# too-z/MultiModalPFN

Hardware: NVIDIA B200
Metric: test rows/sec predict_proba (higher is better)
Workload: dtype bf16

## Files before the change

### multimodalpfn_b200/csrc/common.cuh

```cuda
#pragma once
#include <cuda_bf16.h>
#include <cuda_runtime.h>
#include <stdint.h>

#include <atomic>

#include "../../include/mmpfn_b200.h"

namespace mmpfn {

constexpr int kE = 192;
constexpr int kH = 6;
constexpr int kD = 32;
constexpr int kHid = 768;
constexpr float kLnEps = 1e-5f;

extern std::atomic<int64_t> g_launches;
void set_error(const char* fmt, ...);
int check_geometry(const mmpfn_geometry* g);

inline int count_launch() {
  g_launches.fetch_add(1, std::memory_order_relaxed);
  cudaError_t e = cudaGetLastError();
  if (e != cudaSuccess) {
// ... 4 lines not shown
}

inline int current_device() {
  int d = 0;
  if (cudaGetDevice(&d) != cudaSuccess) { cudaGetLastError(); return -1; }
  return d;
}
inline int device_sm_count() {
  static int n[64] = {0};
  const int d = current_device();
  if (d < 0 || d >= 64) return 148;
  if (!n[d]) {
    int v = 0;
    if (cudaDeviceGetAttribute(&v, cudaDevAttrMultiProcessorCount, d) != cudaSuccess || v < 1) { cudaGetLastError(); v = 148; }
    n[d] = v;
  }
  return n[d];
}
#define MMPFN_OPT_IN_SMEM(kern, bytes)                                                                     \
  do {                                                                                                     \
    static unsigned long long _done = 0;                                                                   \
    const int _d = ::mmpfn::current_device();                                                              \
    if (_d < 0 || _d >= 64 || !((_done >> _d) & 1ull)) {                                                   \
      if (cudaFuncSetAttribute(kern, cudaFuncAttributeMaxDynamicSharedMemorySize, (int)(bytes)) != cudaSuccess) { \
        ::mmpfn::set_error("cannot opt in to %d bytes of dynamic shared memory: %s", (int)(bytes),           \
                           cudaGetErrorString(cudaGetLastError()));                                        \
        return MMPFN_ECUDA;                                                                                \
      }                                                                                                    \
      if (_d >= 0 && _d < 64) _done |= 1ull << _d;                                                         \
    }                                                                                                      \
  } while (0)

#define MMPFN_TRY(expr)            \
  do {                             \
    int _rc = (expr);              \
    if (_rc != MMPFN_OK) return _rc; \
  } while (0)

__device__ __forceinline__ float gelu_exact(float x) {
  return 0.5f * x * (1.0f + erff(x * 0.70710678118654752440f));
}
__device__ __forceinline__ float warp_sum(float v) {
#pragma unroll
  for (int o = 16; o > 0; o >>= 1) v += __shfl_xor_sync(0xffffffffu, v, o);
  return v;
}
__device__ __forceinline__ float warp_max(float v) {
#pragma unroll
  for (int o = 16; o > 0; o >>= 1) v = fmaxf(v, __shfl_xor_sync(0xffffffffu, v, o));
  return v;
}
__device__ __forceinline__ uint32_t pack_bf16x2(float lo, float hi) {
  __nv_bfloat162 v = __floats2bfloat162_rn(lo, hi);
  return *reinterpret_cast<uint32_t*>(&v);
}
__device__ __forceinline__ float fast_exp2f(float x) {
  float y;
  asm("ex2.approx.ftz.f32 %0, %1;" : "=f"(y) : "f"(x));
  return y;
}
__device__ __forceinline__ float bf16_bits_to_float(uint16_t b) { return __uint_as_float(uint32_t(b) << 16); }

enum { EPI_NONE = 0, EPI_GELU = 1, EPI_GLU_PAIR = 2, EPI_ADD_C = 3 };

struct SgemmParams {
  const float* A;
  const float* W;
  const float* bias;
  float* C;
  int M, N, K, lda, ldw, ldc;
  long long a_batch, w_batch, bias_batch, c_batch;
  int batches;
  int row_inner, row_outer;
};
int launch_sgemm(const SgemmParams& p, int epi, cudaStream_t st);

int launch_layernorm(const float* x, const float* res, const float* gamma, const float* beta, long long rows,
                     int width, float* y_f32, uint16_t* y_bf16, cudaStream_t st, long long x_stride = 0);
int launch_kv_extract_f32(const float* qkv, float* kv, int B, int S, int T, cudaStream_t st, const int* n_rows = nullptr);

int launch_feat_attn_f32(const float* qkv, float* att, long long n_seq, int T, cudaStream_t st);
int launch_feat_attn_bf16(const uint16_t* qkv, uint16_t* att, long long n_seq, int T, cudaStream_t st);
bool feat_qkv_attn_supported(int T);
int launch_feat_qkv_attn(const uint16_t* x, const uint16_t* w_qkv, long long M, int T, uint16_t* att, cudaStream_t st);

struct ItemAttnF32 {
  const float *q, *k, *v;
  float* out;
  long long q_outer, q_inner, q_row, kv_outer, kv_inner, kv_row, o_outer, o_inner, o_row;
  int planes, inner, n_q, n_kv, shared_kv;
  const int *q_len, *kv_len;
};
int launch_item_attn_f32(const ItemAttnF32& p, cudaStream_t st);

enum { TC_EPI_BF16 = 0, TC_EPI_GELU_BF16 = 1, TC_EPI_RESID_LN = 2, TC_EPI_QKV_ITEMS = 3, TC_EPI_GLU_PAIR_F32 = 4 };
struct TcGemm {
  const uint16_t* A;
  const uint16_t* W;
  int M, N, K;
  int items;
  int B, S, T;
  int epi;
  uint16_t* out_bf16;
  float* resid_f32;
  uint16_t* ln_bf16;
  uint16_t *q_out, *k_out, *vt_out;
  int S_pad;
  uint16_t *k0_out, *vt0_out;
  const float* bias;
  float* out_f32;
};
int launch_tc_gemm(const TcGemm& p, cudaStream_t st);
int launch_tc_rowgemm(const TcGemm& p, cudaStream_t st);

struct TcMlp {
  const uint16_t* state_b;
  uint16_t* state_b_out;
  float* resid_f32;
  const uint16_t* w1;
  const uint16_t* w2;
  int M;
};
int launch_tc_mlp(const TcMlp& p, cudaStream_t st);

struct TcItemAttn {
  const uint16_t* q;
  const uint16_t* k;
  const uint16_t* vt;
  uint16_t* out;
  int B, T, n_q, Sq_pad, n_kv, Skv_pad;
  int shared_kv;
  int kv_slots;
  long long kv_rank_stride;
  int kv_seg_rows;
  long long kv_seg_stride;
  const int* q_len;
  const int* kv_len;
};
int launch_tc_item_attn(const TcItemAttn& p, cudaStream_t st);

struct TabStatsLayout {
  int Fp, G;
  __host__ __device__ int src() const { return 0; }
  __host__ __device__ int fill() const { return Fp; }
  __host__ __device__ int lo() const { return 2 * Fp; }
  __host__ __device__ int hi() const { return 3 * Fp; }
  __host__ __device__ int mean() const { return 4 * Fp; }
  __host__ __device__ int stdv() const { return 5 * Fp; }
  __host__ __device__ int scale() const { return 6 * Fp; }
  __host__ __device__ int total() const { return 6 * Fp + G; }
};
int launch_tab_fit(const float* x, int B, int S, int F, int fpg, int n_train, float n_sigma, float* stats,
                   cudaStream_t st, const int* n_rows = nullptr, const int* n_train_b = nullptr);
int launch_stem_tokens(const mmpfn_geometry* g, const mmpfn_weights* w, const float* x, const float* stats,
                       const float* img_tok, const float* y, const float* y_mean, const uint64_t* y_mask,
                       const float* pos_emb, int B, int S, int F, int H_img, long long x_bstride, long long y_bstride,
                       long long img_bstride, float* state_f32, uint16_t* state_bf16, int32_t* nan_flag, cudaStream_t st,
                       const long long* img_off = nullptr, const int* n_rows = nullptr);
int launch_cap_attn(const float* kv, const float* q, int S, int n_kv, int Hc, float* out, cudaStream_t st);
int launch_cap_combine(const float* o, const float* ffn, const float* gamma, const float* beta, long long rows,
                       float* out, cudaStream_t st);
int launch_moe_gate_scale(const float* gate_logits, float* tok, int S, int Hm, cudaStream_t st);
int launch_proba_tail(const float* logits, const int32_t* perm, const float* prior, int n_est, int S, int n_out,
                      int n_classes, float temperature, int avg_before, float* proba, cudaStream_t st);

int launch_bar_tail(const float* logits, const float* const* task_logits, const int32_t* row_offset, int n_tasks,
// ... 6 lines not shown
```

### multimodalpfn_b200/csrc/kernels_f32.cu

```cuda
#include "common.cuh"
#include "feat_attn_core.cuh"

namespace mmpfn {

namespace {
constexpr int BM = 128, BN = 64, BK = 16;

template <int EPI>
__global__ void __launch_bounds__(256) sgemm_kernel(SgemmParams p) {
  __shared__ __align__(16) float As[BK][BM + 4];
  __shared__ __align__(16) float Bs[BK][BN + 4];
  const int z = blockIdx.z;
  const float* __restrict__ A = p.A + z * p.a_batch;
  const float* __restrict__ W = p.W + z * p.w_batch;
  const float* __restrict__ bias = p.bias ? p.bias + z * p.bias_batch : nullptr;
  float* __restrict__ C = p.C + z * p.c_batch;
  const int m0 = blockIdx.x * BM, n0 = blockIdx.y * BN;
  const int tid = threadIdx.x;
  const int ty = tid >> 4, tx = tid & 15;

  float acc[8][4];
#pragma unroll
  for (int i = 0; i < 8; ++i)
#pragma unroll
// ... 236 lines not shown
  const int warp = threadIdx.x >> 5, lane = threadIdx.x & 31;
  const int n_kt = (T + 15) >> 4;
  const int Tp = n_kt * 16;
  const uint32_t buf_bytes = (uint32_t)Tp * FA_ROW_BYTES;
  const uint32_t sbase0 = (uint32_t)__cvta_generic_to_shared(fsm);
  constexpr int CH = 3 * kE * 2 / 16;

  auto stage = [&](long long row, int b) {
    const uint8_t* src = reinterpret_cast<const uint8_t*>(qkv + row * T * (3 * kE));
    const uint32_t dst = sbase0 + b * buf_bytes;
    for (int i = threadIdx.x; i < T * CH; i += blockDim.x) {
      const int t = i / CH, c = i % CH;
      asm volatile("cp.async.cg.shared.global [%0], [%1], 16;" ::"r"(dst + t * FA_ROW_BYTES + c * 16),
                   "l"(src + (long long)t * (3 * kE * 2) + c * 16));
    }
    asm volatile("cp.async.commit_group;");
  };
  for (int b = 0; b < n_buf; ++b)
    for (int i = threadIdx.x; i < (Tp - T) * CH; i += blockDim.x) {
      const int t = T + i / CH, c = i % CH;
      *reinterpret_cast<uint4*>(fsm + b * buf_bytes + t * FA_ROW_BYTES + c * 16) = make_uint4(0, 0, 0, 0);
    }
  long long row = blockIdx.x;
  if (row < n_rows) stage(row, 0);
  for (int it = 0; row < n_rows; row += gridDim.x, ++it) {
  const int cur = n_buf == 2 ? (it & 1) : 0;
  const long long nxt = row + gridDim.x;
  if (n_buf == 2 && nxt < n_rows) {
    stage(nxt, cur ^ 1);
    asm volatile("cp.async.wait_group 1;");
  } else {
    asm volatile("cp.async.wait_group 0;");
  }
  __syncthreads();
  const uint32_t sbase = sbase0 + cur * buf_bytes;

  const int n_items = kH * n_kt;
  for (int item = warp; item < n_items; item += (blockDim.x >> 5)) {
    const int h = item / n_kt, mt = item % n_kt;
    feat_attn_item<KT>(sbase, FA_ROW_BYTES, h * kD * 2, (kE + h * kD) * 2, (2 * kE + h * kD) * 2, T, n_kt, mt, lane);
  }
  __syncthreads();
  {
    constexpr int OC = kE * 2 / 16;
    uint8_t* dst = reinterpret_cast<uint8_t*>(att + row * T * kE);
    for (int i = threadIdx.x; i < T * OC; i += blockDim.x) {
      const int t = i / OC, c = i % OC;
      uint4 v;
      asm volatile("ld.shared.v4.b32 {%0, %1, %2, %3}, [%4];" : "=r"(v.x), "=r"(v.y), "=r"(v.z), "=r"(v.w)
                   : "r"(sbase + t * FA_ROW_BYTES + c * 16));
      *reinterpret_cast<uint4*>(dst + (long long)t * (kE * 2) + c * 16) = v;
    }
  }
  __syncthreads();
  if (n_buf == 1 && nxt < n_rows) stage(nxt, 0);
  }
}

template <int KT>
int launch_feat_attn_mma_t(const uint16_t* qkv, uint16_t* att, long long n_seq, int T, cudaStream_t st) {
  const int Tp = (T + 15) / 16 * 16;
  const int n_buf = (size_t)2 * Tp * FA_ROW_BYTES <= 200 * 1024 ? 2 : 1;
  const size_t smem = (size_t)n_buf * Tp * FA_ROW_BYTES;
  auto kern = feat_attn_mma_kernel<KT>;
  MMPFN_OPT_IN_SMEM(kern, 227 * 1024);
  const int n_sm = device_sm_count();
  const int n_items = kH * (Tp / 16);
  const int warps = n_items < 12 ? n_items : 12;
  int per_sm = (int)((227 * 1024) / (smem + 1024));
  if (per_sm > 2048 / (warps * 32)) per_sm = 2048 / (warps * 32);
  if (per_sm < 1) per_sm = 1;
  long long grid = (long long)n_sm * per_sm;
  if (grid > n_seq) grid = n_seq;
  kern<<<(unsigned)grid, warps * 32, smem, st>>>(qkv, att, T, n_seq, n_buf);
  return count_launch();
}
}

int launch_feat_attn_f32(const float* qkv, float* att, long long n_seq, int T, cudaStream_t st) {
  return launch_feat_attn<float, float>(qkv, att, n_seq, T, st);
}
int launch_feat_attn_bf16(const uint16_t* qkv, uint16_t* att, long long n_seq, int T, cudaStream_t st) {
  if (n_seq <= 0) return MMPFN_OK;
  if (T <= 32) return launch_feat_attn_mma_t<2>(qkv, att, n_seq, T, st);
  if (T <= 64) return launch_feat_attn_mma_t<4>(qkv, att, n_seq, T, st);
  if (T <= 96) return launch_feat_attn_mma_t<6>(qkv, att, n_seq, T, st);
  if (T <= 144) return launch_feat_attn_mma_t<9>(qkv, att, n_seq, T, st);
  if (T <= 192) return launch_feat_attn_mma_t<12>(qkv, att, n_seq, T, st);
  return launch_feat_attn<uint16_t, uint16_t>(qkv, att, n_seq, T, st);
}

namespace {
constexpr int IQ = 64, IK = 64;

__global__ void __launch_bounds__(128) item_attn_f32_kernel(ItemAttnF32 p) {
  __shared__ __align__(16) float Qt[kD][IQ];
  __shared__ __align__(16) float Kt[kD][IK];
  __shared__ __align__(16) float Vs[IK][kD];
  __shared__ __align__(16) float Pt[IK][IQ + 4];
  const int plane = blockIdx.z, h = blockIdx.y, q0 = blockIdx.x * IQ;
  const int tid = threadIdx.x;
  const int ty = tid >> 3, tx = tid & 7;
  const int pb = plane / p.inner, pt = plane % p.inner;
  const float* qb = p.q + pb * p.q_outer + pt * p.q_inner + h * kD;
  const int hk = p.shared_kv ? 0 : h;
  const float* kb = p.k + pb * p.kv_outer + pt * p.kv_inner + hk * kD;
  const float* vb = p.v + pb * p.kv_outer + pt * p.kv_inner + hk * kD;
  const int n_q = p.q_len ? min(max(p.q_len[pb], 0), p.n_q) : p.n_q;
  const int n_kv = p.kv_len ? min(max(p.kv_len[pb], 1), p.n_kv) : p.n_kv;
  if (q0 >= n_q) {
    for (int i = tid; i < IQ * (kD / 4); i += 128) {
      const int r = q0 + (i >> 3), c4 = (i & 7) * 4;
      if (r < p.n_q)
        *reinterpret_cast<float4*>(p.out + pb * p.o_outer + pt * p.o_inner + (long long)r * p.o_row + h * kD + c4) =
            make_float4(0.f, 0.f, 0.f, 0.f);
    }
    return;
  }

  const float scale = 0.17677669529663687f;
  for (int i = tid; i < IQ * (kD / 4); i += 128) {
    const int r = i >> 3, c4 = (i & 7) * 4;
    float4 v = make_float4(0, 0, 0, 0);
    if (q0 + r < n_q) v = *reinterpret_cast<const float4*>(qb + (long long)(q0 + r) * p.q_row + c4);
    Qt[c4 + 0][r] = v.x * scale; Qt[c4 + 1][r] = v.y * scale; Qt[c4 + 2][r] = v.z * scale; Qt[c4 + 3][r] = v.w * scale;
  }
  float m[4], l[4], o[4][4];
#pragma unroll
  for (int i = 0; i < 4; ++i) {
    m[i] = -INFINITY;
    l[i] = 0.f;
#pragma unroll
    for (int j = 0; j < 4; ++j) o[i][j] = 0.f;
  }

  for (int k0 = 0; k0 < n_kv; k0 += IK) {
    __syncthreads();
    for (int i = tid; i < IK * (kD / 4); i += 128) {
      const int r = i >> 3, c4 = (i & 7) * 4;
      float4 kv = make_float4(0, 0, 0, 0), vv = kv;
      if (k0 + r < n_kv) {
        kv = *reinterpret_cast<const float4*>(kb + (long long)(k0 + r) * p.kv_row + c4);
        vv = *reinterpret_cast<const float4*>(vb + (long long)(k0 + r) * p.kv_row + c4);
      }
      Kt[c4 + 0][r] = kv.x; Kt[c4 + 1][r] = kv.y; Kt[c4 + 2][r] = kv.z; Kt[c4 + 3][r] = kv.w;
      *reinterpret_cast<float4*>(&Vs[r][c4]) = vv;
    }
    __syncthreads();
    float s[4][8];
#pragma unroll
    for (int i = 0; i < 4; ++i)
#pragma unroll
      for (int j = 0; j < 8; ++j) s[i][j] = 0.f;
#pragma unroll 8
    for (int d = 0; d < kD; ++d) {
      const float4 a = *reinterpret_cast<const float4*>(&Qt[d][ty * 4]);
      const float4 b0 = *reinterpret_cast<const float4*>(&Kt[d][tx * 8]);
      const float4 b1 = *reinterpret_cast<const float4*>(&Kt[d][tx * 8 + 4]);
      const float av[4] = {a.x, a.y, a.z, a.w};
      const float bv[8] = {b0.x, b0.y, b0.z, b0.w, b1.x, b1.y, b1.z, b1.w};
#pragma unroll
      for (int i = 0; i < 4; ++i)
#pragma unroll
        for (int j = 0; j < 8; ++j) s[i][j] = fmaf(av[i], bv[j], s[i][j]);
    }
    float alpha[4];
#pragma unroll
// ... 98 lines not shown
```

### multimodalpfn_b200/csrc/kernels_featfused.cu

```cuda
#include "feat_attn_core.cuh"
#include "tc_common.cuh"

namespace mmpfn {
namespace {

constexpr int U_BM = 128, U_BN = 192, U_K = 192;
constexpr int U_W_BYTES = U_BN * U_K * 2;
constexpr int U_A_BYTES = U_BM * U_K * 2;
constexpr int U_ROW = 2 * 3 * kD * 2 + 16;
constexpr int U_QKV_BYTES = U_BM * U_ROW;
constexpr int U_PAD_ROWS = 12;
constexpr int U_OFF_W = 0;
constexpr int U_OFF_A = U_W_BYTES;
constexpr int U_OFF_QKV = U_OFF_A + U_A_BYTES;
constexpr int U_OFF_BAR = U_OFF_QKV + 2 * U_QKV_BYTES + U_PAD_ROWS * U_ROW;
constexpr int U_SMEM = U_OFF_BAR + 128 + 1024;
constexpr int U_THREADS = 768;
static_assert(U_SMEM <= 227 * 1024, "shared memory budget");
static_assert(U_ROW % 16 == 0 && U_ROW % 128 == 16, "ldmatrix rows: 16-byte aligned, 16 bytes apart modulo 128");

struct FusedArgs {
  uint16_t* att;
  long long M;
  long long n_rows;
// ... 84 lines not shown
#pragma unroll
          for (int k = 0; k < 4; ++k)
            umma_bf16(tmem + ab * U_BN, adesc + (uint64_t)(k * 2), bdesc + (uint64_t)(k * 2), idesc, (kb | k) != 0);
        }
        umma_commit(a_empty);
        umma_commit(&acc_full[ab]);
      }
    }
  } else if (warp >= 4 && warp < 8) {
    const int quarter = warp & 3;
    const int r = quarter * 32 + lane;
    uint32_t v[32];
    for (int i = 0; i < my_tiles; ++i) {
      const int ab = i & 1;
      const uint32_t row = smem_u32(smem) + U_OFF_QKV + ab * U_QKV_BYTES + r * U_ROW;
      const uint32_t trow = tmem + ab * U_BN + ((uint32_t)(quarter * 32) << 16);
      mbar_wait(&acc_full[ab], (i >> 1) & 1);
      tc_fence_after();
#pragma unroll 1
      for (int h2 = 0; h2 < 2; ++h2) {
        mbar_wait(&qkv_empty[ab * 2 + h2], ((i >> 1) & 1) ^ 1);
#pragma unroll 1
        for (int part = 0; part < 3; ++part) {
          const int c = part * 2 + h2;
          tmem_ld32(trow + c * 32, v);
          tmem_ld_wait();
#pragma unroll
          for (int k = 0; k < 4; ++k)
            st_shared_v4(row + c * 64 + k * 16, pack_bf16x2(__uint_as_float(v[8 * k]), __uint_as_float(v[8 * k + 1])),
                         pack_bf16x2(__uint_as_float(v[8 * k + 2]), __uint_as_float(v[8 * k + 3])),
                         pack_bf16x2(__uint_as_float(v[8 * k + 4]), __uint_as_float(v[8 * k + 5])),
                         pack_bf16x2(__uint_as_float(v[8 * k + 6]), __uint_as_float(v[8 * k + 7])));
        }
        mbar_arrive_warp(&qkv_full[ab * 2 + h2]);
      }
      tc_fence_before();
      mbar_arrive_warp(&acc_empty[ab]);
    }
  } else if (warp >= 8) {
    const int h2 = (warp - 8) >> 3, aw = (warp - 8) & 7;
    const int n_kt = (p.T + 15) >> 4;
    for (int i = 0; i < my_tiles; ++i) {
      const int qb = i & 1;
      const uint32_t qbase = smem_u32(smem) + U_OFF_QKV + qb * U_QKV_BYTES;
      const long long row0 = (long long)tile_of(i) * p.G;
      const int g_valid = (int)(p.n_rows - row0 < p.G ? p.n_rows - row0 : p.G);
      mbar_wait(&qkv_full[qb * 2 + h2], (i >> 1) & 1);
      const int n_items = g_valid * n_kt;
      uint8_t* dst = reinterpret_cast<uint8_t*>(p.att + (row0 * p.T) * kE + pair * 64 + h2 * 32);
      for (int item = aw; item < n_items; item += 8) {
        const int g = item / n_kt, mt = item % n_kt;
        const uint32_t rbase = qbase + g * p.T * U_ROW;
        feat_attn_item<KT>(rbase, U_ROW, h2 * 64, 128 + h2 * 64, 256 + h2 * 64, p.T, n_kt, mt, lane);
        __syncwarp();
#pragma unroll
        for (int k = 0; k < 2; ++k) {
          const int idx = lane + 32 * k, t = mt * 16 + (idx >> 2), c = idx & 3;
          if (t < p.T) {
            uint4 o;
            asm volatile("ld.shared.v4.b32 {%0, %1, %2, %3}, [%4];" : "=r"(o.x), "=r"(o.y), "=r"(o.z), "=r"(o.w)
                         : "r"(rbase + t * U_ROW + h2 * 64 + c * 16));
            *reinterpret_cast<uint4*>(dst + (long long)(g * p.T + t) * (kE * 2) + c * 16) = o;
          }
        }
      }
      mbar_arrive_warp(&qkv_empty[qb * 2 + h2]);
    }
  }
  tc_fence_before();
  __syncthreads();
  if (warp == 2) {
    tc_fence_after();
    tmem_dealloc(tmem, 512);
  }
}

template <int KT>
int launch_fused_t(const CUtensorMap& ma, const CUtensorMap& mw, const FusedArgs& a, int grid, cudaStream_t st) {
  MMPFN_OPT_IN_SMEM(feat_qkv_attn_kernel<KT>, U_SMEM);
  feat_qkv_attn_kernel<KT><<<grid, U_THREADS, U_SMEM, st>>>(ma, mw, a);
  return count_launch();
}

}

bool feat_qkv_attn_supported(int T) { return T >= 2 && T <= 64; }

int launch_feat_qkv_attn(const uint16_t* x, const uint16_t* w_qkv, long long M, int T, uint16_t* att, cudaStream_t st) {
  if (M <= 0) return MMPFN_OK;
  if (!feat_qkv_attn_supported(T) || M % T != 0 || M > 2147483647LL) {
    set_error("feat_qkv_attn: unsupported shape (M %lld, T %d)", M, T);
    return MMPFN_EUNSUPPORTED;
  }
  FusedArgs a{};
  a.att = att; a.M = M; a.T = T; a.n_rows = M / T;
  a.G = U_BM / T;
  const int n_kt = (T + 15) / 16;
  while (a.G > 1 && (a.G - 1) * T + 16 * n_kt > U_BM + U_PAD_ROWS) --a.G;
  a.m_tiles = (int)((a.n_rows + a.G - 1) / a.G);
  CUtensorMap ma, mw;
  {
    const cuuint64_t dims[2] = {(cuuint64_t)U_K, (cuuint64_t)M};
    const cuuint64_t strides[1] = {(cuuint64_t)U_K * 2};
    const cuuint32_t box[2] = {64, U_BM};
    MMPFN_TRY(encode_map(&ma, x, 2, dims, strides, box, CU_TENSOR_MAP_SWIZZLE_128B));
  }
  {
    const cuuint64_t dims[2] = {(cuuint64_t)U_K, (cuuint64_t)(3 * kE)};
    const cuuint64_t strides[1] = {(cuuint64_t)U_K * 2};
    const cuuint32_t box[2] = {64, 64};
    MMPFN_TRY(encode_map(&mw, w_qkv, 2, dims, strides, box, CU_TENSOR_MAP_SWIZZLE_128B));
  }
  int per = device_sm_count() / 3;
  if (per > a.m_tiles) per = a.m_tiles;
  if (per < 1) per = 1;
  a.ctas_per_pair = per;
  return T <= 32 ? launch_fused_t<2>(ma, mw, a, per * 3, st) : launch_fused_t<4>(ma, mw, a, per * 3, st);
}

}
```

### multimodalpfn_b200/csrc/tc_common.cuh

```cuda
#pragma once
#include <cuda.h>
#include <stdio.h>
#include <stdlib.h>

#include "common.cuh"

namespace mmpfn {
namespace {

__device__ __forceinline__ uint32_t smem_u32(const void* p) { return (uint32_t)__cvta_generic_to_shared(p); }

__device__ __forceinline__ void mbar_init(uint64_t* bar, uint32_t count) {
  asm volatile("mbarrier.init.shared::cta.b64 [%0], %1;" ::"r"(smem_u32(bar)), "r"(count));
}
__device__ __forceinline__ void mbar_expect_tx(uint64_t* bar, uint32_t bytes) {
  asm volatile("mbarrier.arrive.expect_tx.shared::cta.b64 _, [%0], %1;" ::"r"(smem_u32(bar)), "r"(bytes) : "memory");
}
__device__ __forceinline__ void mbar_arrive(uint64_t* bar) {
  asm volatile("mbarrier.arrive.shared::cta.b64 _, [%0];" ::"r"(smem_u32(bar)) : "memory");
}
__device__ __forceinline__ void mbar_arrive_warp(uint64_t* bar) {
  __syncwarp();
  if ((threadIdx.x & 31) == 0) mbar_arrive(bar);
}
// ... 19 lines not shown
        "bra EXIT_%=;\n\t"
        "DONE_%=:\n\t"
        "mov.u32 %0, 1;\n\t"
        "EXIT_%=:\n\t}"
        : "=r"(done)
        : "r"(addr), "r"(parity), "r"(20000u)
        : "memory");
    if (done) return;
    const long long now = clock64();
    if (t0 == 0) t0 = now;
    else if (now - t0 > 4000000000LL) mbar_timeout();
  }
}
__device__ __forceinline__ bool elect_one() {
  uint32_t pred;
  asm volatile("{\n\t.reg .pred p;\n\telect.sync _|p, 0xffffffff;\n\tselp.u32 %0, 1, 0, p;\n\t}" : "=r"(pred));
  return pred != 0;
}
__device__ __forceinline__ bool mbar_test(uint64_t* bar, uint32_t parity) {
  uint32_t done;
  asm volatile(
      "{\n\t.reg .pred p;\n\t"
      "mbarrier.test_wait.parity.shared::cta.b64 p, [%1], %2;\n\t"
      "selp.u32 %0, 1, 0, p;\n\t}"
      : "=r"(done)
      : "r"(smem_u32(bar)), "r"(parity)
      : "memory");
  return done != 0;
}
__device__ __forceinline__ void mbar_wait2(uint64_t* bar_a, uint32_t parity_a, uint64_t* bar_b, uint32_t parity_b) {
  const uint32_t a = smem_u32(bar_a), b = smem_u32(bar_b);
  uint32_t n = 0;
  long long t0 = 0;
  while (true) {
    uint32_t da, db;
    asm volatile(
        "{\n\t.reg .pred p, q;\n\t"
        "mbarrier.try_wait.parity.shared::cta.b64 p, [%2], %3, %6;\n\t"
        "mbarrier.try_wait.parity.shared::cta.b64 q, [%4], %5, %6;\n\t"
        "selp.u32 %0, 1, 0, p;\n\t"
        "selp.u32 %1, 1, 0, q;\n\t}"
        : "=r"(da), "=r"(db)
        : "r"(a), "r"(parity_a), "r"(b), "r"(parity_b), "r"(20000u)
        : "memory");
    if (da & db) return;
    if ((++n & 4095u) == 0) {
      const long long now = clock64();
      if (t0 == 0) t0 = now;
      else if (now - t0 > 4000000000LL) mbar_timeout();
    }
  }
}
__device__ __forceinline__ void fence_barrier_init() { asm volatile("fence.mbarrier_init.release.cluster;" ::: "memory"); }
__device__ __forceinline__ void fence_proxy_async() { asm volatile("fence.proxy.async.shared::cta;" ::: "memory"); }
__device__ __forceinline__ void tc_fence_before() { asm volatile("tcgen05.fence::before_thread_sync;" ::: "memory"); }
__device__ __forceinline__ void tc_fence_after() { asm volatile("tcgen05.fence::after_thread_sync;" ::: "memory"); }

__device__ __forceinline__ void tma_load_2d(void* dst, const CUtensorMap* map, uint64_t* bar, int c0, int c1) {
  asm volatile(
      "cp.async.bulk.tensor.2d.shared::cluster.global.mbarrier::complete_tx::bytes [%0], [%1, {%3, %4}], [%2];"
      ::"r"(smem_u32(dst)), "l"(map), "r"(smem_u32(bar)), "r"(c0), "r"(c1)
      : "memory");
}
__device__ __forceinline__ void tma_load_3d(void* dst, const CUtensorMap* map, uint64_t* bar, int c0, int c1, int c2) {
  asm volatile(
      "cp.async.bulk.tensor.3d.shared::cluster.global.mbarrier::complete_tx::bytes [%0], [%1, {%3, %4, %5}], [%2];"
      ::"r"(smem_u32(dst)), "l"(map), "r"(smem_u32(bar)), "r"(c0), "r"(c1), "r"(c2)
      : "memory");
}
__device__ __forceinline__ void tma_load_4d(void* dst, const CUtensorMap* map, uint64_t* bar, int c0, int c1, int c2,
                                            int c3) {
  asm volatile(
      "cp.async.bulk.tensor.4d.shared::cluster.global.mbarrier::complete_tx::bytes [%0], [%1, {%3, %4, %5, %6}], [%2];"
      ::"r"(smem_u32(dst)), "l"(map), "r"(smem_u32(bar)), "r"(c0), "r"(c1), "r"(c2), "r"(c3)
      : "memory");
}
__device__ __forceinline__ void tma_load_5d(void* dst, const CUtensorMap* map, uint64_t* bar, int c0, int c1, int c2,
                                            int c3, int c4) {
  asm volatile(
      "cp.async.bulk.tensor.5d.shared::cluster.global.mbarrier::complete_tx::bytes [%0], [%1, {%3, %4, %5, %6, %7}], [%2];"
      ::"r"(smem_u32(dst)), "l"(map), "r"(smem_u32(bar)), "r"(c0), "r"(c1), "r"(c2), "r"(c3), "r"(c4)
      : "memory");
}
__device__ __forceinline__ void l2_prefetch(const void* gptr, uint32_t bytes) {
  asm volatile("cp.async.bulk.prefetch.L2.global [%0], %1;" ::"l"(gptr), "r"(bytes) : "memory");
}
__device__ __forceinline__ void prefetch_tmap(const CUtensorMap* map) {
  asm volatile("prefetch.tensormap [%0];" ::"l"(map) : "memory");
}

__device__ __forceinline__ void tmem_alloc(uint32_t* dst_smem, uint32_t ncols) {
  asm volatile("tcgen05.alloc.cta_group::1.sync.aligned.shared::cta.b32 [%0], %1;" ::"r"(smem_u32(dst_smem)), "r"(ncols)
               : "memory");
  asm volatile("tcgen05.relinquish_alloc_permit.cta_group::1.sync.aligned;" ::: "memory");
}
__device__ __forceinline__ void tmem_dealloc(uint32_t taddr, uint32_t ncols) {
  asm volatile("tcgen05.dealloc.cta_group::1.sync.aligned.b32 %0, %1;" ::"r"(taddr), "r"(ncols) : "memory");
}
__device__ __forceinline__ void umma_bf16(uint32_t d_tmem, uint64_t adesc, uint64_t bdesc, uint32_t idesc,
                                          uint32_t accumulate) {
  asm volatile(
      "{\n\t.reg .pred p;\n\t"
      "setp.ne.b32 p, %4, 0;\n\t"
      "tcgen05.mma.cta_group::1.kind::f16 [%0], %1, %2, %3, p;\n\t}"
      ::"r"(d_tmem), "l"(adesc), "l"(bdesc), "r"(idesc), "r"(accumulate)
      : "memory");
}
__device__ __forceinline__ void umma_bf16_ts(uint32_t d_tmem, uint32_t a_tmem, uint64_t bdesc, uint32_t idesc,
                                             uint32_t accumulate) {
  asm volatile(
      "{\n\t.reg .pred p;\n\t"
      "setp.ne.b32 p, %4, 0;\n\t"
      "tcgen05.mma.cta_group::1.kind::f16 [%0], [%1], %2, %3, p;\n\t}"
      ::"r"(d_tmem), "r"(a_tmem), "l"(bdesc), "r"(idesc), "r"(accumulate)
      : "memory");
}
__device__ __forceinline__ void umma_commit(uint64_t* bar) {
  asm volatile("tcgen05.commit.cta_group::1.mbarrier::arrive::one.shared::cluster.b64 [%0];" ::"r"(smem_u32(bar))
               : "memory");
}
__device__ __forceinline__ void tmem_ld32(uint32_t taddr, uint32_t (&v)[32]) {
  asm volatile(
      "tcgen05.ld.sync.aligned.32x32b.x32.b32 "
      "{%0, %1, %2, %3, %4, %5, %6, %7, %8, %9, %10, %11, %12, %13, %14, %15, "
      "%16, %17, %18, %19, %20, %21, %22, %23, %24, %25, %26, %27, %28, %29, %30, %31}, [%32];"
      : "=r"(v[0]), "=r"(v[1]), "=r"(v[2]), "=r"(v[3]), "=r"(v[4]), "=r"(v[5]), "=r"(v[6]), "=r"(v[7]), "=r"(v[8]),
        "=r"(v[9]), "=r"(v[10]), "=r"(v[11]), "=r"(v[12]), "=r"(v[13]), "=r"(v[14]), "=r"(v[15]), "=r"(v[16]),
        "=r"(v[17]), "=r"(v[18]), "=r"(v[19]), "=r"(v[20]), "=r"(v[21]), "=r"(v[22]), "=r"(v[23]), "=r"(v[24]),
        "=r"(v[25]), "=r"(v[26]), "=r"(v[27]), "=r"(v[28]), "=r"(v[29]), "=r"(v[30]), "=r"(v[31])
      : "r"(taddr)
      : "memory");
}
__device__ __forceinline__ void tmem_ld16(uint32_t taddr, uint32_t (&v)[16]) {
  asm volatile(
      "tcgen05.ld.sync.aligned.32x32b.x16.b32 "
      "{%0, %1, %2, %3, %4, %5, %6, %7, %8, %9, %10, %11, %12, %13, %14, %15}, [%16];"
      : "=r"(v[0]), "=r"(v[1]), "=r"(v[2]), "=r"(v[3]), "=r"(v[4]), "=r"(v[5]), "=r"(v[6]), "=r"(v[7]), "=r"(v[8]),
        "=r"(v[9]), "=r"(v[10]), "=r"(v[11]), "=r"(v[12]), "=r"(v[13]), "=r"(v[14]), "=r"(v[15])
      : "r"(taddr)
      : "memory");
}
__device__ __forceinline__ void tmem_ld_wait() { asm volatile("tcgen05.wait::ld.sync.aligned;" ::: "memory"); }
__device__ __forceinline__ void tmem_st32(uint32_t taddr, const uint32_t (&v)[32]) {
  asm volatile(
      "tcgen05.st.sync.aligned.32x32b.x32.b32 [%0], "
      "{%1, %2, %3, %4, %5, %6, %7, %8, %9, %10, %11, %12, %13, %14, %15, %16, "
      "%17, %18, %19, %20, %21, %22, %23, %24, %25, %26, %27, %28, %29, %30, %31, %32};"
      ::"r"(taddr), "r"(v[0]), "r"(v[1]), "r"(v[2]), "r"(v[3]), "r"(v[4]), "r"(v[5]), "r"(v[6]), "r"(v[7]), "r"(v[8]),
        "r"(v[9]), "r"(v[10]), "r"(v[11]), "r"(v[12]), "r"(v[13]), "r"(v[14]), "r"(v[15]), "r"(v[16]), "r"(v[17]),
        "r"(v[18]), "r"(v[19]), "r"(v[20]), "r"(v[21]), "r"(v[22]), "r"(v[23]), "r"(v[24]), "r"(v[25]), "r"(v[26]),
        "r"(v[27]), "r"(v[28]), "r"(v[29]), "r"(v[30]), "r"(v[31])
      : "memory");
}
__device__ __forceinline__ void tmem_st_wait() { asm volatile("tcgen05.wait::st.sync.aligned;" ::: "memory"); }

__device__ __forceinline__ float fast_exp2(float x) {
  float y;
  asm("ex2.approx.ftz.f32 %0, %1;" : "=f"(y) : "f"(x));
  return y;
}

__device__ __forceinline__ float poly_exp2(float x) {
  x = fminf(fmaxf(x, -126.0f), 126.0f);
  const float r = x + 12582912.0f;
  const float f = x - (r - 12582912.0f);
  float p = fmaf(0.05520550534129143f, f, 0.24261397123336792f);
  p = fmaf(p, f, 0.6932547688484192f);
  p = fmaf(p, f, 0.9999276995658875f);
  return __uint_as_float(__float_as_uint(p) + (__float_as_uint(r) << 23));
}
__host__ __device__ constexpr bool poly_sel(int i, int PN) { return ((i + 1) * PN) / 32 != (i * PN) / 32; }

__device__ __forceinline__ uint64_t pack_f32x2(float lo, float hi) {
  uint64_t r;
  asm("mov.b64 %0, {%1, %2};" : "=l"(r) : "f"(lo), "f"(hi));
  return r;
}
__device__ __forceinline__ void unpack_f32x2(uint64_t v, float& lo, float& hi) {
  asm("mov.b64 {%0, %1}, %2;" : "=f"(lo), "=f"(hi) : "l"(v));
}
__device__ __forceinline__ uint64_t fma_f32x2(uint64_t a, uint64_t b, uint64_t c) {
  uint64_t r;
  asm("fma.rn.f32x2 %0, %1, %2, %3;" : "=l"(r) : "l"(a), "l"(b), "l"(c));
  return r;
}
__device__ __forceinline__ uint64_t add_f32x2(uint64_t a, uint64_t b) {
  uint64_t r;
  asm("add.rn.f32x2 %0, %1, %2;" : "=l"(r) : "l"(a), "l"(b));
  return r;
}

__device__ __forceinline__ void st_shared_v4(uint32_t saddr, uint32_t a, uint32_t b, uint32_t c, uint32_t d) {
  asm volatile("st.shared.v4.b32 [%0], {%1, %2, %3, %4};" ::"r"(saddr), "r"(a), "r"(b), "r"(c), "r"(d) : "memory");
}

__device__ __forceinline__ void tma_store_2d(const CUtensorMap* map, const void* src, int c0, int c1) {
  asm volatile("cp.async.bulk.tensor.2d.global.shared::cta.bulk_group [%0, {%2, %3}], [%1];"
               ::"l"(map), "r"(smem_u32(src)), "r"(c0), "r"(c1) : "memory");
}
__device__ __forceinline__ void tma_store_3d(const CUtensorMap* map, const void* src, int c0, int c1, int c2) {
  asm volatile("cp.async.bulk.tensor.3d.global.shared::cta.bulk_group [%0, {%2, %3, %4}], [%1];"
               ::"l"(map), "r"(smem_u32(src)), "r"(c0), "r"(c1), "r"(c2) : "memory");
}
__device__ __forceinline__ void st_shared_u16(uint32_t saddr, uint16_t v) {
  asm volatile("st.shared.u16 [%0], %1;" ::"r"(saddr), "h"(v) : "memory");
}
__device__ __forceinline__ void bulk_commit() { asm volatile("cp.async.bulk.commit_group;" ::: "memory"); }
__device__ __forceinline__ void bulk_wait_read0() { asm volatile("cp.async.bulk.wait_group.read 0;" ::: "memory"); }
__device__ __forceinline__ void bulk_wait0() { asm volatile("cp.async.bulk.wait_group 0;" ::: "memory"); }
__device__ __forceinline__ void epi_bar() { asm volatile("bar.sync 1, 128;" ::: "memory"); }

__device__ __forceinline__ float4 lds128(uint32_t saddr) {
  float4 v;
  asm volatile("ld.shared.v4.f32 {%0, %1, %2, %3}, [%4];" : "=f"(v.x), "=f"(v.y), "=f"(v.z), "=f"(v.w) : "r"(saddr));
  return v;
}

constexpr uint32_t kSw128 = 2, kSw64 = 4;
__device__ __forceinline__ uint64_t make_desc(uint32_t saddr, uint32_t sbo_bytes, uint32_t layout) {
  uint64_t d = 0;
  d |= (uint64_t)((saddr & 0x3FFFFu) >> 4);
  d |= (uint64_t)1 << 16;
  d |= (uint64_t)(sbo_bytes >> 4) << 32;
  d |= (uint64_t)1 << 46;
  d |= (uint64_t)layout << 61;
  return d;
}
__host__ __device__ constexpr uint32_t make_idesc(int M, int N) {
  return (1u << 4) | (1u << 7) | (1u << 10) | ((uint32_t)(N >> 3) << 17) | ((uint32_t)(M >> 4) << 24);
}


typedef CUresult (*EncodeTiledFn)(CUtensorMap*, CUtensorMapDataType, cuuint32_t, void*, const cuuint64_t*,
                                  const cuuint64_t*, const cuuint32_t*, const cuuint32_t*, CUtensorMapInterleave,
// ... 36 lines not shown
```

Before: 9721.

## Add warp-specialized tcgen05 feature-attention kernel for short feature sequences

Adds a new warp-specialized kernel for T<=32 feature attention. It uses TMA loads, tcgen05 UMMA for QK^T and PV with the scores kept in TMEM, and softmax warps that write bf16 P back into TMEM. It optionally fuses the QKV projection GEMM, pipelined against the attention. The kernel replaces both the mma.sync path for T<=32 and the previous fused QKV+attention kernel, and packs 4 sequences per 128-row tile. The aim is higher tensor core throughput and overlap of loading, projection and attention, at the cost of much added complexity and possible correctness risk in the descriptor and layout handling.

New measurement: 9679, median of 6. Within noise of the previous version (-0.4%).

```diff
diff --git a/multimodalpfn_b200/csrc/common.cuh b/multimodalpfn_b200/csrc/common.cuh
--- a/multimodalpfn_b200/csrc/common.cuh
+++ b/multimodalpfn_b200/csrc/common.cuh
@@ -110,6 +110,7 @@
 int launch_feat_attn_f32(const float* qkv, float* att, long long n_seq, int T, cudaStream_t st);
 int launch_feat_attn_bf16(const uint16_t* qkv, uint16_t* att, long long n_seq, int T, cudaStream_t st);
 bool feat_qkv_attn_supported(int T);
+int launch_feat_attn_tc(const uint16_t* qkv, uint16_t* att, long long n_rows, int T, cudaStream_t st);
 int launch_feat_qkv_attn(const uint16_t* x, const uint16_t* w_qkv, long long M, int T, uint16_t* att, cudaStream_t st);
 
 struct ItemAttnF32 {
diff --git a/multimodalpfn_b200/csrc/kernels_f32.cu b/multimodalpfn_b200/csrc/kernels_f32.cu
--- a/multimodalpfn_b200/csrc/kernels_f32.cu
+++ b/multimodalpfn_b200/csrc/kernels_f32.cu
@@ -342,7 +342,7 @@
 }
 int launch_feat_attn_bf16(const uint16_t* qkv, uint16_t* att, long long n_seq, int T, cudaStream_t st) {
   if (n_seq <= 0) return MMPFN_OK;
-  if (T <= 32) return launch_feat_attn_mma_t<2>(qkv, att, n_seq, T, st);
+  if (T <= 32) return launch_feat_attn_tc(qkv, att, n_seq, T, st);
   if (T <= 64) return launch_feat_attn_mma_t<4>(qkv, att, n_seq, T, st);
   if (T <= 96) return launch_feat_attn_mma_t<6>(qkv, att, n_seq, T, st);
   if (T <= 144) return launch_feat_attn_mma_t<9>(qkv, att, n_seq, T, st);
diff --git a/multimodalpfn_b200/csrc/kernels_featfused.cu b/multimodalpfn_b200/csrc/kernels_featfused.cu
--- a/multimodalpfn_b200/csrc/kernels_featfused.cu
+++ b/multimodalpfn_b200/csrc/kernels_featfused.cu
@@ -190,15 +190,328 @@
   return count_launch();
 }
 
+constexpr int V_G = 4;
+constexpr int V_BLK = U_BM * kD * 2;
+constexpr int V_QKV_BYTES = 6 * V_BLK;
+#ifndef FEAT_TC_PF
+#define FEAT_TC_PF 1
+#endif
+#ifndef FEAT_TC_NQ
+#define FEAT_TC_NQ 2
+#endif
+constexpr int V_NQ = FEAT_TC_NQ;
+constexpr int V_OFF_BAR = U_OFF_A + 3 * U_A_BYTES;
+constexpr int V_SMEM = V_OFF_BAR + 256 + 1024;
+constexpr int V_THREADS = 640;
+constexpr int V_TM_S = U_BN, V_TM_HEAD = V_G * 32 + kD;
+static_assert(V_SMEM <= 227 * 1024, "shared memory budget");
+static_assert(V_TM_S + 2 * V_TM_HEAD <= 512, "TMEM budget");
+
+struct TcArgs {
+  uint16_t* att;
+  long long n_rows;
+  int T, m_tiles, ctas_per_pair;
+};
+
+__device__ __forceinline__ uint64_t make_desc_mn64(uint32_t saddr) {
+  return (make_desc(saddr, 512, kSw64) & ~(0x3FFFull << 16)) | ((uint64_t)(512 >> 4) << 16);
+}
+
+template <bool FROM_QKV>
+__global__ void __launch_bounds__(V_THREADS, 1) feat_attn_tc_kernel(const __grid_constant__ CUtensorMap map_in,
+                                                                   const __grid_constant__ CUtensorMap map_w,
+                                                                   const TcArgs p) {
+  extern __shared__ uint8_t smem_raw[];
+  uint8_t* smem = (uint8_t*)(((uintptr_t)smem_raw + 1023) & ~(uintptr_t)1023);
+  uint64_t* bars = (uint64_t*)(smem + V_OFF_BAR);
+  uint64_t* w_full = bars;
+  uint64_t* a_full = bars + 1;
+  uint64_t* a_empty = bars + 3;
+  uint64_t* acc_full = bars + 5;
+  uint64_t* acc_empty = bars + 6;
+  uint64_t* qkv_full = bars + 7;
+  uint64_t* qkv_empty = bars + 11;
+  uint64_t* s_full = bars + 15;
+  uint64_t* p_full = bars + 17;
+  uint64_t* o_full = bars + 19;
+  uint32_t* tmem_slot = (uint32_t*)(bars + 21);
+  constexpr int NQ = FROM_QKV ? 2 : V_NQ, NA = 3 - NQ;
+  constexpr int OFF_QKV = U_OFF_A + NA * U_A_BYTES;
+
+  const int warp = threadIdx.x >> 5, lane = threadIdx.x & 31;
+  const int pair = (int)blockIdx.x % 3;
+  const int cid = (int)blockIdx.x / 3;
+  const int my_tiles = cid < p.m_tiles ? (p.m_tiles - cid + p.ctas_per_pair - 1) / p.ctas_per_pair : 0;
+  auto tile_of = [&](int i) { return cid + i * p.ctas_per_pair; };
+  const uint32_t sq = smem_u32(smem) + OFF_QKV;
+
+  if (threadIdx.x == 0) {
+    prefetch_tmap(&map_in);
+    if (!FROM_QKV) prefetch_tmap(&map_w);
+    mbar_init(w_full, 1);
+    for (int s = 0; s < 2; ++s) {
+      mbar_init(&a_full[s], 1);
+      mbar_init(&a_empty[s], 1);
+    }
+    mbar_init(acc_full, 1);
+    mbar_init(acc_empty, 8);
+    for (int s = 0; s < 4; ++s) {
+      mbar_init(&qkv_full[s], FROM_QKV ? 1 : 4);
+      mbar_init(&qkv_empty[s], 1);
+    }
+    for (int h = 0; h < 2; ++h) {
+      mbar_init(&s_full[h], 1);
+      mbar_init(&p_full[h], 4);
+      mbar_init(&o_full[h], 1);
+    }
+    fence_barrier_init();
+  }
+  if (warp == 2) tmem_alloc(tmem_slot, 512);
+  tc_fence_before();
+  __syncthreads();
+  tc_fence_after();
+  const uint32_t tmem = *tmem_slot;
+
+  if (warp == 0) {
+    if (elect_one()) {
+      if constexpr (FROM_QKV) {
+        for (int i = 0; i < my_tiles; ++i) {
+          const int b = i % NQ, row0 = tile_of(i) * V_G;
+          for (int h2 = 0; h2 < 2; ++h2) {
+            mbar_wait(&qkv_empty[b * 2 + h2], ((i / NQ) & 1) ^ 1);
+            mbar_expect_tx(&qkv_full[b * 2 + h2], 3 * V_BLK);
+#pragma unroll
+            for (int part = 0; part < 3; ++part)
+              tma_load_3d(smem + OFF_QKV + b * V_QKV_BYTES + (h2 * 3 + part) * V_BLK, &map_in, &qkv_full[b * 2 + h2],
+                          part * kE + pair * 64 + h2 * kD, 0, row0);
+          }
+        }
+      } else {
+        mbar_expect_tx(w_full, U_W_BYTES);
+#pragma unroll
+        for (int kb = 0; kb < 3; ++kb)
+#pragma unroll
+          for (int part = 0; part < 3; ++part)
+            tma_load_2d(smem + U_OFF_W + kb * (U_BN * 128) + part * (64 * 128), &map_w, w_full, kb * 64,
+                        part * kE + pair * 64);
+        for (int i = 0; i < my_tiles; ++i) {
+          const int sa = i % NA;
+          mbar_wait(&a_empty[sa], ((i / NA) & 1) ^ 1);
+          mbar_expect_tx(&a_full[sa], U_A_BYTES);
+#pragma unroll
+          for (int kb = 0; kb < 3; ++kb)
+            tma_load_3d(smem + U_OFF_A + sa * U_A_BYTES + kb * (U_BM * 128), &map_in, &a_full[sa], kb * 64, 0,
+                        tile_of(i) * V_G);
+          if (FEAT_TC_PF > 0 && i + FEAT_TC_PF < my_tiles)
+#pragma unroll
+            for (int kb = 0; kb < 3; ++kb) tma_prefetch_3d(&map_in, kb * 64, 0, tile_of(i + FEAT_TC_PF) * V_G);
+        }
+      }
+    }
+  } else if (warp == 1) {
+    if (elect_one()) {
+      constexpr uint32_t idesc_qkv = make_idesc(U_BM, U_BN);
+      constexpr uint32_t idesc_s = make_idesc(U_BM, V_G * 32);
+      constexpr uint32_t idesc_o = make_idesc(U_BM, kD) | (1u << 16);
+      const uint32_t sbase = smem_u32(smem);
+      auto issue_qkv = [&](int j) {
+        const int sa = j % NA;
+        mbar_wait(&a_full[sa], (j / NA) & 1);
+        mbar_wait(acc_empty, (j & 1) ^ 1);
+        tc_fence_after();
+#pragma unroll
+        for (int kb = 0; kb < 3; ++kb) {
+          const uint64_t adesc = make_desc(sbase + U_OFF_A + sa * U_A_BYTES + kb * (U_BM * 128), 1024, kSw128);
+          const uint64_t bdesc = make_desc(sbase + U_OFF_W + kb * (U_BN * 128), 1024, kSw128);
+#pragma unroll
+          for (int k = 0; k < 4; ++k)
+            umma_bf16(tmem, adesc + (uint64_t)(k * 2), bdesc + (uint64_t)(k * 2), idesc_qkv, (kb | k) != 0);
+        }
+        umma_commit(&a_empty[sa]);
+        umma_commit(acc_full);
+      };
+      if (!FROM_QKV) {
+        mbar_wait(w_full, 0);
+        if (my_tiles > 0) issue_qkv(0);
+      }
+      for (int i = 0; i < my_tiles; ++i) {
+        const int b = i % NQ;
+#pragma unroll 1
+        for (int h2 = 0; h2 < 2; ++h2) {
+          mbar_wait(&qkv_full[b * 2 + h2], (i / NQ) & 1);
+          tc_fence_after();
+          const uint32_t blk = sq + b * V_QKV_BYTES + h2 * 3 * V_BLK;
+          const uint64_t qdesc = make_desc(blk, 512, kSw64), kdesc = make_desc(blk + V_BLK, 512, kSw64);
+#pragma unroll
+          for (int k = 0; k < kD / 16; ++k)
+            umma_bf16(tmem + V_TM_S + h2 * V_TM_HEAD, qdesc + (uint64_t)(k * 2), kdesc + (uint64_t)(k * 2), idesc_s, k != 0);
+          umma_commit(&s_full[h2]);
+        }
+        if (!FROM_QKV && i + 1 < my_tiles) issue_qkv(i + 1);
+#pragma unroll 1
+        for (int h2 = 0; h2 < 2; ++h2) {
+          mbar_wait(&p_full[h2], i & 1);
+          tc_fence_after();
+          const uint32_t ts = tmem + V_TM_S + h2 * V_TM_HEAD;
+          const uint64_t vdesc = make_desc_mn64(sq + b * V_QKV_BYTES + (h2 * 3 + 2) * V_BLK);
+#pragma unroll
+          for (int k = 0; k < V_G * 32 / 16; ++k)
+            umma_bf16_ts(ts + V_G * 32, ts + k * 8, vdesc + (uint64_t)(k * 64), idesc_o, k != 0);
+          umma_commit(&qkv_empty[b * 2 + h2]);
+          umma_commit(&o_full[h2]);
+        }
+      }
+    }
+  } else if (warp >= 4 && warp < 12) {
+    if constexpr (!FROM_QKV) {
+      const int h2 = (warp - 4) >> 2, quarter = warp & 3;
+      const int r = quarter * 32 + lane;
+      const uint32_t tcol = tmem + ((uint32_t)(quarter * 32) << 16) + h2 * 32;
+      const uint32_t sw = (r >> 1) & 3;
+      auto store_row = [&](uint32_t row, const uint32_t (&v)[32]) {
+#pragma unroll
+        for (int k = 0; k < 4; ++k)
+          st_shared_v4(row + ((k ^ sw) << 4), pack_bf16x2(__uint_as_float(v[8 * k]), __uint_as_float(v[8 * k + 1])),
+                       pack_bf16x2(__uint_as_float(v[8 * k + 2]), __uint_as_float(v[8 * k + 3])),
+                       pack_bf16x2(__uint_as_float(v[8 * k + 4]), __uint_as_float(v[8 * k + 5])),
+                       pack_bf16x2(__uint_as_float(v[8 * k + 6]), __uint_as_float(v[8 * k + 7])));
+      };
+      uint32_t va[32], vb[32];
+      for (int i = 0; i < my_tiles; ++i) {
+        const int b = i % NQ;
+        const uint32_t row = sq + b * V_QKV_BYTES + h2 * 3 * V_BLK + r * 64;
+        mbar_wait(&qkv_empty[b * 2 + h2], ((i / NQ) & 1) ^ 1);
+        mbar_wait(acc_full, i & 1);
+        tc_fence_after();
+        tmem_ld32(tcol, va);
+        tmem_ld_wait();
+        tmem_ld32(tcol + 64, vb);
+        store_row(row, va);
+        tmem_ld_wait();
+        tmem_ld32(tcol + 128, va);
+        store_row(row + V_BLK, vb);
+        tmem_ld_wait();
+        tc_fence_before();
+        mbar_arrive_warp(acc_empty);
+        store_row(row + 2 * V_BLK, va);
+        fence_proxy_async();
+        mbar_arrive_warp(&qkv_full[b * 2 + h2]);
+      }
+    }
+  } else if (warp >= 12) {
+    const int h2 = (warp - 12) >> 2, g = warp & 3;
+    const uint32_t ts = tmem + V_TM_S + h2 * V_TM_HEAD + ((uint32_t)(g * 32) << 16);
+    const float c2 = 0.17677669529663687f * 1.4426950408889634f;
+    uint32_t zero[16];
+#pragma unroll
+    for (int j = 0; j < 16; ++j) zero[j] = 0u;
+    for (int i = 0; i < my_tiles; ++i) {
+      const long long row = (long long)tile_of(i) * V_G + g;
+      uint32_t s[32];
+      mbar_wait(&s_full[h2], i & 1);
+      tc_fence_after();
+      tmem_ld32(ts + g * 32, s);
+      tmem_ld_wait();
+      float mx = -INFINITY;
+#pragma unroll
+      for (int j = 0; j < 32; ++j) {
+        if (j >= p.T) s[j] = __float_as_uint(-INFINITY);
+        mx = fmaxf(mx, __uint_as_float(s[j]));
+      }
+      const float mc = mx * c2;
+      float l = 0.f;
+      uint32_t pk[16];
+#pragma unroll
+      for (int j = 0; j < 16; ++j) {
+        const float p0 = fast_exp2f(fmaf(__uint_as_float(s[2 * j]), c2, -mc));
+        const float p1 = fast_exp2f(fmaf(__uint_as_float(s[2 * j + 1]), c2, -mc));
+        l += p0 + p1;
+        pk[j] = pack_bf16x2(p0, p1);
+      }
+      tmem_st16(ts + g * 16, pk);
+#pragma unroll
+      for (int c = 1; c < 4; ++c) tmem_st16(ts + ((g + c) & 3) * 16, zero);
+      tmem_st_wait();
+      tc_fence_before();
+      mbar_arrive_warp(&p_full[h2]);
+      mbar_wait(&o_full[h2], i & 1);
+      tc_fence_after();
+      uint32_t o[32];
+      tmem_ld32(ts + V_G * 32, o);
+      tmem_ld_wait();
+      if (lane < p.T && row < p.n_rows) {
+        const float inv = 1.0f / l;
+        uint4* d4 = reinterpret_cast<uint4*>(p.att + (row * p.T + lane) * kE + pair * 64 + h2 * kD);
+#pragma unroll
+        for (int k = 0; k < 4; ++k)
+          d4[k] = make_uint4(pack_bf16x2(__uint_as_float(o[8 * k]) * inv, __uint_as_float(o[8 * k + 1]) * inv),
+                             pack_bf16x2(__uint_as_float(o[8 * k + 2]) * inv, __uint_as_float(o[8 * k + 3]) * inv),
+                             pack_bf16x2(__uint_as_float(o[8 * k + 4]) * inv, __uint_as_float(o[8 * k + 5]) * inv),
+                             pack_bf16x2(__uint_as_float(o[8 * k + 6]) * inv, __uint_as_float(o[8 * k + 7]) * inv));
+      }
+    }
+    tc_fence_before();
+  }
+  __syncthreads();
+  if (warp == 2) {
+    tc_fence_after();
+    tmem_dealloc(tmem, 512);
+  }
+}
+
+template <bool FROM_QKV>
+int launch_tc_t(const CUtensorMap& mi, const CUtensorMap& mw, long long n_rows, int T, uint16_t* att, cudaStream_t st) {
+  TcArgs a{};
+  a.att = att; a.n_rows = n_rows; a.T = T;
+  a.m_tiles = (int)((n_rows + V_G - 1) / V_G);
+  int per = device_sm_count() / 3;
+  if (per > a.m_tiles) per = a.m_tiles;
+  if (per < 1) per = 1;
+  a.ctas_per_pair = per;
+  MMPFN_OPT_IN_SMEM(feat_attn_tc_kernel<FROM_QKV>, V_SMEM);
+  feat_attn_tc_kernel<FROM_QKV><<<per * 3, V_THREADS, V_SMEM, st>>>(mi, mw, a);
+  return count_launch();
+}
+
+int encode_rows_map(CUtensorMap* m, const uint16_t* base, int cols, long long n_rows, int T, int box_cols,
+                    CUtensorMapSwizzle sw) {
+  const cuuint64_t dims[3] = {(cuuint64_t)cols, (cuuint64_t)T, (cuuint64_t)n_rows};
+  const cuuint64_t strides[2] = {(cuuint64_t)cols * 2, (cuuint64_t)T * cols * 2};
+  const cuuint32_t box[3] = {(cuuint32_t)box_cols, 32, V_G};
+  return encode_map(m, base, 3, dims, strides, box, sw);
+}
+
 }
 
 bool feat_qkv_attn_supported(int T) { return T >= 2 && T <= 64; }
+
+int launch_feat_attn_tc(const uint16_t* qkv, uint16_t* att, long long n_rows, int T, cudaStream_t st) {
+  if (n_rows <= 0) return MMPFN_OK;
+  if (T < 1 || T > 32 || n_rows > 2147483647LL / 4) {
+    set_error("feat_attn_tc: unsupported shape (rows %lld, T %d)", n_rows, T);
+    return MMPFN_EUNSUPPORTED;
+  }
+  CUtensorMap mq;
+  MMPFN_TRY(encode_rows_map(&mq, qkv, 3 * kE, n_rows, T, kD, CU_TENSOR_MAP_SWIZZLE_64B));
+  return launch_tc_t<true>(mq, mq, n_rows, T, att, st);
+}
 
 int launch_feat_qkv_attn(const uint16_t* x, const uint16_t* w_qkv, long long M, int T, uint16_t* att, cudaStream_t st) {
   if (M <= 0) return MMPFN_OK;
   if (!feat_qkv_attn_supported(T) || M % T != 0 || M > 2147483647LL) {
     set_error("feat_qkv_attn: unsupported shape (M %lld, T %d)", M, T);
     return MMPFN_EUNSUPPORTED;
+  }
+  CUtensorMap ma, mw;
+  {
+    const cuuint64_t dims[2] = {(cuuint64_t)U_K, (cuuint64_t)(3 * kE)};
+    const cuuint64_t strides[1] = {(cuuint64_t)U_K * 2};
+    const cuuint32_t box[2] = {64, 64};
+    MMPFN_TRY(encode_map(&mw, w_qkv, 2, dims, strides, box, CU_TENSOR_MAP_SWIZZLE_128B));
+  }
+  if (T <= 32) {
+    MMPFN_TRY(encode_rows_map(&ma, x, U_K, M / T, T, 64, CU_TENSOR_MAP_SWIZZLE_128B));
+    return launch_tc_t<false>(ma, mw, M / T, T, att, st);
   }
   FusedArgs a{};
   a.att = att; a.M = M; a.T = T; a.n_rows = M / T;
@@ -206,24 +519,17 @@
   const int n_kt = (T + 15) / 16;
   while (a.G > 1 && (a.G - 1) * T + 16 * n_kt > U_BM + U_PAD_ROWS) --a.G;
   a.m_tiles = (int)((a.n_rows + a.G - 1) / a.G);
-  CUtensorMap ma, mw;
   {
     const cuuint64_t dims[2] = {(cuuint64_t)U_K, (cuuint64_t)M};
     const cuuint64_t strides[1] = {(cuuint64_t)U_K * 2};
     const cuuint32_t box[2] = {64, U_BM};
     MMPFN_TRY(encode_map(&ma, x, 2, dims, strides, box, CU_TENSOR_MAP_SWIZZLE_128B));
   }
-  {
-    const cuuint64_t dims[2] = {(cuuint64_t)U_K, (cuuint64_t)(3 * kE)};
-    const cuuint64_t strides[1] = {(cuuint64_t)U_K * 2};
-    const cuuint32_t box[2] = {64, 64};
-    MMPFN_TRY(encode_map(&mw, w_qkv, 2, dims, strides, box, CU_TENSOR_MAP_SWIZZLE_128B));
-  }
   int per = device_sm_count() / 3;
   if (per > a.m_tiles) per = a.m_tiles;
   if (per < 1) per = 1;
   a.ctas_per_pair = per;
-  return T <= 32 ? launch_fused_t<2>(ma, mw, a, per * 3, st) : launch_fused_t<4>(ma, mw, a, per * 3, st);
-}
-
-}
+  return launch_fused_t<4>(ma, mw, a, per * 3, st);
+}
+
+}
diff --git a/multimodalpfn_b200/csrc/tc_common.cuh b/multimodalpfn_b200/csrc/tc_common.cuh
--- a/multimodalpfn_b200/csrc/tc_common.cuh
+++ b/multimodalpfn_b200/csrc/tc_common.cuh
@@ -125,6 +125,10 @@
       ::"r"(smem_u32(dst)), "l"(map), "r"(smem_u32(bar)), "r"(c0), "r"(c1), "r"(c2), "r"(c3), "r"(c4)
       : "memory");
 }
+__device__ __forceinline__ void tma_prefetch_3d(const CUtensorMap* map, int c0, int c1, int c2) {
+  asm volatile("cp.async.bulk.prefetch.tensor.3d.L2.global.tile [%0, {%1, %2, %3}];" ::"l"(map), "r"(c0), "r"(c1), "r"(c2)
+               : "memory");
+}
 __device__ __forceinline__ void l2_prefetch(const void* gptr, uint32_t bytes) {
   asm volatile("cp.async.bulk.prefetch.L2.global [%0], %1;" ::"l"(gptr), "r"(bytes) : "memory");
 }
@@ -193,6 +197,14 @@
         "r"(v[9]), "r"(v[10]), "r"(v[11]), "r"(v[12]), "r"(v[13]), "r"(v[14]), "r"(v[15]), "r"(v[16]), "r"(v[17]),
         "r"(v[18]), "r"(v[19]), "r"(v[20]), "r"(v[21]), "r"(v[22]), "r"(v[23]), "r"(v[24]), "r"(v[25]), "r"(v[26]),
         "r"(v[27]), "r"(v[28]), "r"(v[29]), "r"(v[30]), "r"(v[31])
+      : "memory");
+}
+__device__ __forceinline__ void tmem_st16(uint32_t taddr, const uint32_t (&v)[16]) {
+  asm volatile(
+      "tcgen05.st.sync.aligned.32x32b.x16.b32 [%0], "
+      "{%1, %2, %3, %4, %5, %6, %7, %8, %9, %10, %11, %12, %13, %14, %15, %16};"
+      ::"r"(taddr), "r"(v[0]), "r"(v[1]), "r"(v[2]), "r"(v[3]), "r"(v[4]), "r"(v[5]), "r"(v[6]), "r"(v[7]), "r"(v[8]),
+        "r"(v[9]), "r"(v[10]), "r"(v[11]), "r"(v[12]), "r"(v[13]), "r"(v[14]), "r"(v[15])
       : "memory");
 }
 __device__ __forceinline__ void tmem_st_wait() { asm volatile("tcgen05.wait::st.sync.aligned;" ::: "memory"); }
```
